# Dao-AILab/flash-attention

Measured on AMD Instinct MI355X. Metric: attention_fwd_tflops, higher is better.
Workload: dtype bf16; 1 GPU; BASELINE config 3: B=4 H=32 S=4096 D=128 bf16 causal, forward (flash_attn_func path, fa_fwd via C ABI); batch=4, heads=32, seqlen=4096, head_dim=128, causal=True, parallelism=replicas x1

## Files before the change

### flash-attention_amd/csrc/fa_api.cpp

```cpp
#include <hip/hip_runtime.h>
#include <dlfcn.h>

#include <algorithm>
#include <atomic>
#include <cmath>
#include <cstdarg>
#include <cstdio>
#include <cstdlib>
#include <cstring>
#include <initializer_list>

#include "../../include/fa_gfx950.h"
#include "fa_device.h"
#include "fa_kernel_params.h"
#include "fa_launch.h"

namespace {

thread_local char g_err[512] = {0};

int fail(int code, const char* fmt, ...) {
  va_list ap;
  va_start(ap, fmt);
  vsnprintf(g_err, sizeof(g_err), fmt, ap);
  va_end(ap);
  return code;
}

int env_int(const char* name, int dflt) {
  const char* s = getenv(name);
  return (s && *s) ? atoi(s) : dflt;
}

std::atomic<const fa::Knobs*> g_knobs{nullptr};
const fa::Knobs* read_knobs() {
  fa::Knobs* k = new fa::Knobs();
  k->fwd_nw = env_int("FA_FWD_NW", 0);
  const char* t = getenv("FA_RESCALE_THR");
  k->rescale_thr = (t && *t) ? (float)atof(t) : 8.f;
  if (!(k->rescale_thr >= 0.f) || k->rescale_thr > 16.f) k->rescale_thr = 0.f;
  k->varlen_list = env_int("FA_VARLEN_LIST", 1);
  k->il_sched = env_int("FA_IL_SCHED", 3);
  k->bwd_dq_nw = env_int("FA_BWD_DQ_NW", 0);
  k->bwd_mode = env_int("FA_BWD_MODE", 0);
  k->bwd_dkdv = env_int("FA_BWD_DKDV", 0);
  k->bwd_ds_cap_mb = env_int("FA_BWD_DS_CAP_MB", 8192);
  k->bwd_fused_check = env_int("FA_BWD_FUSED_CHECK", 0);
  k->bwd_c5_cap_mb = std::max(16, std::min(65536, env_int("FA_BWD_C5_CAP_MB", 1024)));
  k->fz_line = std::max(1, std::min(64, env_int("FA_FZ_LINE", 32)));
  k->bwd_gsplit = env_int("FA_BWD_GSPLIT", 1);
  k->w64_persist = env_int("FA_W64_PERSIST", 1);
  k->strict = env_int("FA_STRICT", 0);
  k->dkdv_prescale = env_int("FA_DKDV_PRESCALE", 0);
  k->bwd_fuse_delta = env_int("FA_BWD_FUSE_DELTA", 1);
  k->pack_gqa = env_int("FA_PACK_GQA", 1);
  k->fp8_kv_ring = env_int("FA_FP8_KV_RING", 4);
  if (k->fp8_kv_ring < 2 || k->fp8_kv_ring > 4) k->fp8_kv_ring = 4;
  k->launch_log = env_int("FA_DEBUG_LAUNCH_LOG", 0);
  if (k->strict) k->rescale_thr = 0.f;
  return k;
}

}
namespace fa {
const Knobs& knobs() {
  const Knobs* k = g_knobs.load(std::memory_order_acquire);
  if (!k) {
    const Knobs* fresh = read_knobs();
    if (g_knobs.compare_exchange_strong(k, fresh, std::memory_order_acq_rel)) k = fresh;
    else delete fresh;
  }
  return *k;
}
LastSchedule& last_schedule() {
  thread_local LastSchedule ls{};
  return ls;
}
namespace {
constexpr int kLaunchLogCap = 256;
struct LaunchLog { int n; const void* kern[kLaunchLogCap]; };
LaunchLog& launch_log() {
  thread_local LaunchLog l{};
  return l;
}
}
void launch_log_push(const void* kern) {
  LaunchLog& l = launch_log();
  if (l.n < kLaunchLogCap) l.kern[l.n] = kern;
  ++l.n;
}
void launch_log_clear() { launch_log().n = 0; }
int launch_log_count() { return launch_log().n; }
const void* launch_log_at(int i) { return (i >= 0 && i < launch_log().n && i < kLaunchLogCap) ? launch_log().kern[i] : nullptr; }
}
namespace {

bool head_dim_trimmed(int d) { return d == 32 || d == 96 || d == 192; }
bool head_dim_native(int d) { return d == 64 || d == 128 || d == 256 || head_dim_trimmed(d); }
int head_dim_kernel(int d) { for (int n : {32, 64, 96, 128, 192}) if (d <= n) return n; return 256; }
int head_dim_pitch(int d) { return d <= 64 ? 64 : d <= 128 ? 128 : 256; }

void normalize_window(int seqlen_q, int seqlen_k, bool has_alibi, int& is_causal, int& wl, int& wr) {
  if (wl >= seqlen_k) wl = -1;
  if (wr >= seqlen_k) wr = -1;
  if (seqlen_q == 1 && !has_alibi) is_causal = 0;
  if (is_causal) wr = 0;
  if (wl < 0) wl = -1;
  if (wr < 0) wr = -1;
}

int check_dropout(float p_dropout, const void* rng_state) {
  if (!(p_dropout >= 0.f) || p_dropout >= 1.f) return fail(FA_ERR_INVALID_ARGUMENT, "p_dropout must be in [0, 1)");
  if (p_dropout > 0.f && !rng_state) return fail(FA_ERR_INVALID_ARGUMENT, "p_dropout > 0 needs a device rng_state {seed, offset}");
  return FA_OK;
}
template <typename K> void fill_dropout(K& k, float p_dropout, const uint64_t* rng_state, int seqlen_k) {
  if (p_dropout > 0.f) {
    k.rng = rng_state;
    const float p_keep = 1.0f - p_dropout;
    k.drop_thr8 = (uint32_t)std::floor(p_keep * 255.0f);
    k.rp_keep = 1.f / (1.f - p_dropout);
  }
}

inline bool mla_pair(int d, int d_v) { return d == 576 && d_v == 512; }
constexpr int kMlaBlockRows = 64;
int pack_group(const FaFwdParams* a) {
  const int g = a->h_k > 0 ? a->h / a->h_k : 1;
  if (mla_pair(a->d, a->d_v)) return g > 1 ? g : 1;
  if (g <= 1 || !fa::knobs().pack_gqa || (a->d_v > 0 && a->d_v != a->d) || a->cu_seqlens_q || a->seqused_q || a->p_dropout > 0.f || a->seqlen_q < 1 || (long)a->seqlen_q * g > 128) return 1;
  return g;
}
int choose_splits(const FaFwdParams* a, int& split_tiles) {
  const int tiles = (a->seqlen_k + 63) / 64;
// ... 1076 lines not shown
```

### flash-attention_amd/csrc/fa_fwd_w64.hip

```cpp
#include <cstddef>
#include <cstdio>
#include <cstdlib>
#include <type_traits>

#include "fa_device.h"
#include "fa_kernel_params.h"
#include "fa_launch.h"
#include "fa_fwd_w64_regs.h"
#define FA_W64_CLOB FA_W64_ACC_CLOBBERS
#include "fa_w64_asm.h"


#define FA_W64_AH 3
#define FA_W64_KDMA_G0 0
#define FA_W64_KDMA_GS 2
#define FA_W64_VDMA_G0 1
#define FA_W64_VDMA_GS 2

namespace fa {

template <int D> FA_DEVINL constexpr int k_swz_w(int row) { return D == 128 ? (row & 15) : ((row >> 1) & 7); }
template <int D> FA_DEVINL constexpr int v_swz_w(int row) { return D == 128 ? (row & 3) : ((row >> 1) & 1); }

#define FA_W64_MFMA(E_) (std::is_same<E_, __bf16>::value ? "v_mfma_f32_32x32x16_bf16" : "v_mfma_f32_32x32x16_f16")
constexpr int W64_Q_BASE = 128;
template <typename E, int F> FA_DEVINL void mfma_s_first(f32x16& d, u32x4 a, const f32x16& c) {
  if constexpr (std::is_same<E, __bf16>::value)
    asm volatile("v_mfma_f32_32x32x16_bf16 %0, %1, a[%c3:%c4], %2" : "=&v"(d) : "v"(a), "v"(c), "i"(W64_Q_BASE + 4 * F), "i"(W64_Q_BASE + 4 * F + 3) : FA_W64_ACC_CLOBBERS);
  else
    asm volatile("v_mfma_f32_32x32x16_f16 %0, %1, a[%c3:%c4], %2" : "=&v"(d) : "v"(a), "v"(c), "i"(W64_Q_BASE + 4 * F), "i"(W64_Q_BASE + 4 * F + 3) : FA_W64_ACC_CLOBBERS);
}
template <typename E, int F> FA_DEVINL void mfma_s_acc(f32x16& d, u32x4 a) {
  if constexpr (std::is_same<E, __bf16>::value)
    asm volatile("v_mfma_f32_32x32x16_bf16 %0, %1, a[%c2:%c3], %0" : "+v"(d) : "v"(a), "i"(W64_Q_BASE + 4 * F), "i"(W64_Q_BASE + 4 * F + 3) : FA_W64_ACC_CLOBBERS);
  else
    asm volatile("v_mfma_f32_32x32x16_f16 %0, %1, a[%c2:%c3], %0" : "+v"(d) : "v"(a), "i"(W64_Q_BASE + 4 * F), "i"(W64_Q_BASE + 4 * F + 3) : FA_W64_ACC_CLOBBERS);
}
template <typename E, int T> FA_DEVINL void mfma_o_acc(u32x4 a, u32x4 b) {
  if constexpr (std::is_same<E, __bf16>::value)
    asm volatile("v_mfma_f32_32x32x16_bf16 a[%c2:%c3], %0, %1, a[%c2:%c3]" : : "v"(a), "v"(b), "i"(16 * T), "i"(16 * T + 15) : FA_W64_ACC_CLOBBERS);
  else
    asm volatile("v_mfma_f32_32x32x16_f16 a[%c2:%c3], %0, %1, a[%c2:%c3]" : : "v"(a), "v"(b), "i"(16 * T), "i"(16 * T + 15) : FA_W64_ACC_CLOBBERS);
}
template <typename E, int D, int FEAT = 0, bool PAGED = false, bool DENSE = false>
__global__ void __launch_bounds__(256, 1) fa_fwd_w64_kernel(const FwdK p) {
  constexpr bool ALIBI = FEAT == FEAT_ALIBI;
  static_assert(!PAGED || FEAT == 0, "the paged variant serves plain attention");
  static_assert(!DENSE || (FEAT == 0 && !PAGED), "the dense variant serves plain attention on contiguous keys / values");
  constexpr bool SOFTCAP = FEAT == FEAT_CAP;
  constexpr bool DROP = FEAT == FEAT_DROP;
  constexpr bool DESC = ALIBI;
  static_assert(FEAT == 0 || FEAT == FEAT_ALIBI || FEAT == FEAT_CAP || FEAT == FEAT_DROP, "feature variants of this schedule: none, causal ALiBi, softcap, dropout");
  using T = ElemTraits<E>;
  using V8 = typename T::v8;
  constexpr int NW = 4, QB = 2, BM = NW * 64, BN = 64, CPR = D / 8;
  constexpr int ROW_BYTES = D * 2;
  constexpr int TILE_BYTES = BN * ROW_BYTES;
  constexpr int KS = D / 16;
  constexpr int DB = D / 32;
  static_assert(D == 64 || D == 128, "head dims built natively: 64, 128");
  constexpr float kLn2 = 0.6931471805599453f;

  extern __shared__ __attribute__((aligned(16))) char smem[];
  char FA_LDS* lds = (char FA_LDS*)smem;
  constexpr int STAGE_BYTES = BM * (ROW_BYTES + 16);
  constexpr int Q_OFF = (4 * TILE_BYTES > STAGE_BYTES ? 4 * TILE_BYTES : STAGE_BYTES + 1023) / 1024 * 1024;

  const int tid = threadIdx.x;
  const int lane = tid & 63;
  const int wave = __builtin_amdgcn_readfirstlane(tid >> 6);
  const int hi = lane >> 5, qi = lane & 31;

  const int d_row = lane / CPR, d_pc = lane % CPR;
  constexpr int RPD = 1024 / ROW_BYTES;

  struct Blk { int b, h, m_block, sq, sk; int64_t q_row0, k_row0, q_boff, k_boff, v_boff, o_boff; };
  const int n_virtual = p.persist_total > 0 ? p.persist_total : (int)gridDim.x;
  auto load_rc = [&]() __attribute__((always_inline)) {
#if defined(__HIP_DEVICE_COMPILE__)
    const char __attribute__((address_space(4)))* ka = (const char __attribute__((address_space(4)))*)__builtin_amdgcn_kernarg_segment_ptr();
    asm volatile("" : "+s"(ka));
    const uint32_t __attribute__((address_space(4)))* w = (const uint32_t __attribute__((address_space(4)))*)(ka + offsetof(FwdK, rc));
    W64Rc r;
    r.mul[0] = w[0]; r.mul[1] = w[1]; r.mul[2] = w[2]; r.mul[3] = w[3]; r.mul[4] = w[4]; r.shifts = w[5];
    return r;
#else
    return p.rc;
#endif
  };
  const W64Rc rc0 = load_rc();
  const int g8 = (int)(gridDim.x >> 3);
  const bool snake = p.persist_total > 0 && p.wr >= 0 && p.unit_size > 1 && g8 - fastdiv(g8, rc_get(rc0, RC_UNIT)) * p.unit_size == 0;
  auto decode_id = [&](const W64Rc& rc, int vb, int round, Blk& k) __attribute__((always_inline)) -> bool {
    if (vb >= n_virtual) return false;
    if (!DENSE && p.work_list) {
      if (!work_list_item(p.work_list, vb, p.h, p.h_k, k.b, k.h, k.m_block)) return false;
    } else {
      if (!fwd_w64_decode(p, rc, vb, snake && (round & 1), k.b, k.h, k.m_block)) return false;
    }
    return true;
  };
  auto fill_blk = [&](Blk& k) __attribute__((always_inline)) -> bool {
    k.sq = p.sq; k.sk = p.sk; k.q_row0 = 0; k.k_row0 = 0;
    if constexpr (DENSE) {
      k.q_boff = (int64_t)k.b * p.q_bs; k.k_boff = (int64_t)k.b * p.k_bs; k.v_boff = (int64_t)k.b * p.v_bs; k.o_boff = (int64_t)k.b * p.o_bs;
      return k.m_block * BM < k.sq;
    }
    const int bkv = p.kv_batch_idx ? p.kv_batch_idx[k.b] : k.b;
    k.q_boff = (int64_t)k.b * p.q_bs; k.k_boff = (int64_t)bkv * p.k_bs; k.v_boff = (int64_t)bkv * p.v_bs; k.o_boff = (int64_t)k.b * p.o_bs;
    if (p.cu_q) { const int c0 = p.cu_q[k.b]; k.sq = p.cu_q[k.b + 1] - c0; k.q_row0 = c0; k.q_boff = 0; k.o_boff = 0; }
    if (p.seqused_q) k.sq = min(k.sq, p.seqused_q[k.b]);
    if (p.cu_k) { const int c0 = p.cu_k[k.b]; k.sk = p.cu_k[k.b + 1] - c0; k.k_row0 = c0; k.k_boff = 0; k.v_boff = 0; }
    if (p.seqused_k) k.sk = min(p.seqused_k[k.b] + p.seqused_add, (p.cu_k && !PAGED) ? k.sk : p.sk);
    if (p.leftpad_k) {
      const int lp = p.leftpad_k[k.b];
      k.sk = max(0, k.sk - lp);
      k.k_row0 += lp;
    }
    if constexpr (PAGED) { k.k_boff = 0; k.v_boff = 0; k.k_row0 = 0; }
    return k.m_block * BM < k.sq;
  };
  constexpr int QDMA = (BM * ROW_BYTES) / 1024 / NW;
  auto q_srd_of = [&](const Blk& k) __attribute__((always_inline)) {
    const E* base = (const E*)p.q + k.q_boff + (k.q_row0 + (int64_t)k.m_block * BM) * p.q_rs + (int64_t)k.h * p.q_hs;
    const int rows = min(BM, k.sq - k.m_block * BM);
    const unsigned long long a = (unsigned long long)base;
    const unsigned nrec = rows > 0 ? (unsigned)(((unsigned long long)(rows - 1) * (unsigned long long)p.q_rs + D) * 2ull) : 0u;
    const unsigned lo = __builtin_amdgcn_readfirstlane((unsigned)a);
    const unsigned hi16 = __builtin_amdgcn_readfirstlane((unsigned)(a >> 32)) & 0xffffu;
    const unsigned nr = __builtin_amdgcn_readfirstlane(nrec);
    u32x4 srd = {lo, hi16, nr, 0x00020000u};
    return srd;
  };
  auto dma_q_piece = [&](const u32x4& srd, int i) __attribute__((always_inline)) {
    const int pc = wave * QDMA + i;
    const int row = pc * RPD + d_row;
    const unsigned vo = (unsigned)(row * (int)p.q_rs + ((d_pc ^ k_swz_w<D>(row)) << 3)) * 2u;
    const unsigned dst = __builtin_amdgcn_readfirstlane((unsigned)(Q_OFF + pc * 1024));
    unsigned keep;
    asm volatile("s_mov_b32 %0, m0\n\ts_mov_b32 m0, %2\n\ts_nop 0\n\tbuffer_load_dwordx4 %1, %3, 0 offen lds\n\ts_mov_b32 m0, %0"
                 : "=&s"(keep) : "v"(vo), "s"(dst), "s"(srd) : "memory");
  };
  auto dma_q = [&](const u32x4& srd) __attribute__((always_inline)) {
#pragma unroll 1
    for (int i = 0; i < QDMA; ++i) dma_q_piece(srd, i);
  };
  int q_in_lds = -1;

  constexpr int NDMA = TILE_BYTES / 1024;
  constexpr int DPW = NDMA / NW;
  unsigned koff_l[DPW], voff_l[DPW];
#pragma unroll
  for (int i = 0; i < DPW; ++i) {
    const int row = (wave * DPW + i) * RPD + d_row;
    const int kc = d_pc ^ k_swz_w<D>(row);
    const int vc = ((((d_pc >> 2) ^ v_swz_w<D>(row)) << 2) | (d_pc & 3));
    koff_l[i] = (unsigned)(row * (int)p.k_rs + kc * 8) * 2u - (unsigned)(i * 1024);
    voff_l[i] = (unsigned)(row * (int)p.v_rs + vc * 8) * 2u - (unsigned)(i * 1024);
  }
  const float thr = p.rescale_thr;
  const bool has_wl = !DENSE && p.wl >= 0;

  Blk cur_id;
  cur_id.b = 0; cur_id.h = 0; cur_id.m_block = 0;
  bool cur_ok = decode_id(rc0, (int)blockIdx.x, 0, cur_id);
  for (int vb = blockIdx.x, round = 0; vb < n_virtual; vb += gridDim.x, ++round) {
  Blk blk = cur_id, nxt;
  const bool blk_ok = cur_ok && fill_blk(blk);
  nxt.b = 0; nxt.h = 0; nxt.m_block = 0;
  const W64Rc rc = load_rc();
  const bool nxt_id_ok = p.persist_total > 0 && decode_id(rc, vb + (int)gridDim.x, round + 1, nxt);
  cur_id.b = __builtin_amdgcn_readfirstlane(nxt.b); cur_id.h = __builtin_amdgcn_readfirstlane(nxt.h); cur_id.m_block = __builtin_amdgcn_readfirstlane(nxt.m_block);
  cur_ok = nxt_id_ok;
  if (!blk_ok) continue;
  const int b = blk.b, h = blk.h, m_block = blk.m_block, sq = blk.sq, sk = blk.sk;
  const int hk = fastdiv(h, rc_get(rc, RC_HKR));
  const int64_t q_row0 = blk.q_row0, k_row0 = blk.k_row0, q_boff = blk.q_boff, k_boff = blk.k_boff, v_boff = blk.v_boff, o_boff = blk.o_boff;
  const int m0 = m_block * BM;

  const E* __restrict__ kp = (const E*)p.k + k_boff + k_row0 * p.k_rs + (int64_t)hk * p.k_hs;
  const E* __restrict__ vp = (const E*)p.v + v_boff + k_row0 * p.v_rs + (int64_t)hk * p.v_hs;
  E* __restrict__ op = (E*)p.o + o_boff + q_row0 * p.o_rs + (int64_t)h * p.o_hs;
  float* __restrict__ lsep = (!DENSE && p.cu_q) ? (p.lse + (int64_t)h * p.total_q + q_row0) : (p.lse + ((int64_t)b * p.h + h) * p.sq);

  const int shift = sk - sq;
  const int blk_last = min(m0 + BM, sq) - 1;
  int kmax = sk - 1, kmin = 0;
  if (p.wr >= 0) kmax = min(kmax, blk_last + shift + p.wr);
  if (has_wl) kmin = max(0, m0 + shift - p.wl);
  const int n_min = kmin / BN;
  const int n_max = (kmax >= kmin) ? (kmax / BN + 1) : n_min;
  const int n_tiles = n_max - n_min;
  const int n_steps = 2 * n_tiles;
  const int key_base = n_min * BN;
  auto tile_of = [&](int u) __attribute__((always_inline)) { return DESC ? n_tiles - 1 - u : u; };
  auto step_key = [&](int i) __attribute__((always_inline)) { return key_base + BN * tile_of(i >> 1) + 32 * (i & 1); };
  float slope2 = 0.f;
  if constexpr (ALIBI) slope2 = p.alibi[(int64_t)b * p.alibi_bs + h] * 1.4426950408889634f;

  const int w_row0 = m0 + wave * 64;
  const int w_row1 = min(w_row0 + 63, sq - 1);
  const bool wave_valid = w_row0 < sq;
  const int w_kmax = (p.wr >= 0) ? min(sk - 1, w_row1 + shift + p.wr) : sk - 1;
  const int w_kmin = has_wl ? max(0, w_row0 + shift - p.wl) : 0;
  const int w_full_hi = (p.wr >= 0) ? min(sk - 1, w_row0 + shift + p.wr) : sk - 1;
  const int w_full_lo = has_wl ? (w_row1 + shift - p.wl) : 0;
  int lim_hi[QB], lim_lo[QB];
#pragma unroll
  for (int qb = 0; qb < QB; ++qb) {
    const int my_row = w_row0 + 32 * qb + qi;
    lim_hi[qb] = (p.wr >= 0) ? min(sk - 1, my_row + shift + p.wr) : sk - 1;
    lim_lo[qb] = has_wl ? max(0, my_row + shift - p.wl) : 0;
  }
  auto make_srd = [&](const void* base, int64_t row_stride) __attribute__((always_inline)) {
    const unsigned long long a = (unsigned long long)base;
    const unsigned lo = __builtin_amdgcn_readfirstlane((unsigned)a);
    const unsigned hi16 = __builtin_amdgcn_readfirstlane((unsigned)(a >> 32)) & 0xffffu;
    const unsigned long long bytes = sk > 0 ? ((unsigned long long)(sk - 1) * (unsigned long long)row_stride + D) * 2ull : 0ull;
    const unsigned nrec = __builtin_amdgcn_readfirstlane((unsigned)(bytes > 0xffffffffull ? 0xffffffffull : bytes));
    u32x4 s = {lo, hi16, nrec, 0x00020000u};
    return s;
  };
  const u32x4 k_srd = make_srd(kp, p.k_rs), v_srd = make_srd(vp, p.v_rs);
  const u32x4 null_srd = {k_srd[0], k_srd[1], 0u, k_srd[3]};
  const int pg_tpp = __builtin_amdgcn_readfirstlane(PAGED ? p.page_size / BN : 1);
  const int pg_last = __builtin_amdgcn_readfirstlane(sk > 0 ? (sk - 1) / max(p.page_size, 1) : 0);
  const int* __restrict__ pg_table = p.block_table + (PAGED ? (int64_t)__builtin_amdgcn_readfirstlane(b) * p.block_table_bs : 0);
  auto page_entry = [&](int page) __attribute__((always_inline)) {
    const int pc = min(max(page, 0), pg_last);
    return __builtin_amdgcn_readfirstlane(pg_table[pc]);
  };
  const unsigned pg_bytes_k = (unsigned)__builtin_amdgcn_readfirstlane((int)(unsigned)(p.k_bs * 2)), pg_bytes_v = (unsigned)__builtin_amdgcn_readfirstlane((int)(unsigned)(p.v_bs * 2));
  const unsigned tl_bytes_k = (unsigned)__builtin_amdgcn_readfirstlane((int)(unsigned)(BN * p.k_rs * 2)), tl_bytes_v = (unsigned)__builtin_amdgcn_readfirstlane((int)(unsigned)(BN * p.v_rs * 2));
  auto uniform64 = [](const void* ptr) __attribute__((always_inline)) {
    const unsigned long long a = (unsigned long long)ptr;
    const unsigned lo = (unsigned)__builtin_amdgcn_readfirstlane((int)(unsigned)a), hi = (unsigned)__builtin_amdgcn_readfirstlane((int)(unsigned)(a >> 32));
    return ((unsigned long long)hi << 32) | (unsigned long long)lo;
  };
  const unsigned long long pg_base_k = uniform64(kp), pg_base_v = uniform64(vp);
  auto tile_srd = [&](auto isvc, int blk, int tin, int n) __attribute__((always_inline)) {
    constexpr bool ISV = decltype(isvc)::value != 0;
    const unsigned rs = (unsigned)(ISV ? p.v_rs : p.k_rs);
    const int rows = (n >= 0) ? min(BN, sk - n * BN) : 0;
    const unsigned long long a = (ISV ? pg_base_v : pg_base_k) + (unsigned long long)(unsigned)blk * (unsigned long long)(ISV ? pg_bytes_v : pg_bytes_k) + (unsigned long long)((unsigned)tin * (ISV ? tl_bytes_v : tl_bytes_k));
    const unsigned nrec = rows > 0 ? ((unsigned)(rows - 1) * rs + (unsigned)D) * 2u : 0u;
    u32x4 sd = {(unsigned)a, (unsigned)(a >> 32) & 0xffffu, nrec, 0x00020000u};
    return sd;
  };
  auto dma_pieces = [&](const u32x4& srd, const unsigned (&vo)[DPW], unsigned lds_dst) __attribute__((always_inline)) {
    unsigned keep;
    const unsigned dst = __builtin_amdgcn_readfirstlane(lds_dst);
    if constexpr (DPW == 4) {
      asm volatile("s_mov_b32 %0, m0\n\ts_mov_b32 m0, %5\n\ts_nop 0\n\t"
                   "buffer_load_dwordx4 %1, %6, 0 offen lds\n\t"
                   "buffer_load_dwordx4 %2, %6, 0 offen offset:1024 lds\n\t"
                   "buffer_load_dwordx4 %3, %6, 0 offen offset:2048 lds\n\t"
                   "buffer_load_dwordx4 %4, %6, 0 offen offset:3072 lds\n\t"
                   "s_mov_b32 m0, %0"
                   : "=&s"(keep) : "v"(vo[0]), "v"(vo[1]), "v"(vo[2]), "v"(vo[3]), "s"(dst), "s"(srd) : "memory");
    } else {
      asm volatile("s_mov_b32 %0, m0\n\ts_mov_b32 m0, %3\n\ts_nop 0\n\t"
                   "buffer_load_dwordx4 %1, %4, 0 offen lds\n\t"
                   "buffer_load_dwordx4 %2, %4, 0 offen offset:1024 lds\n\t"
                   "s_mov_b32 m0, %0"
                   : "=&s"(keep) : "v"(vo[0]), "v"(vo[DPW - 1]), "s"(dst), "s"(srd) : "memory");
    }
  };
  auto dma_tile = [&](auto isvc, int buf, int t) __attribute__((always_inline)) {
    constexpr bool ISV = decltype(isvc)::value != 0;
    const bool real = t >= 0 && t < n_tiles;
    const int64_t rs = ISV ? p.v_rs : p.k_rs;
    const unsigned lds_dst = (unsigned)((ISV ? 2 + buf : buf) * TILE_BYTES + wave * DPW * 1024);
    if constexpr (PAGED) {
      const int n = n_min + t, page = max(n, 0) / pg_tpp;
      const u32x4 sd = real ? tile_srd(isvc, page_entry(page), max(n, 0) - page * pg_tpp, n) : null_srd;
      dma_pieces(sd, ISV ? voff_l : koff_l, lds_dst);
      return;
    }
// ... 318 lines not shown
          cap_a1[e] = __builtin_fmaf(yv, kCapTiny, capoff[e >> 4]);
          cap_d[e] = fast_exp2(yv) + 1.f;
        }
      }
#pragma unroll
      for (int e = (DO_P ? el_end(x) : 32); e < (DO_P ? el_end(x + 1) : 32); ++e) {
        const int eq = e >> 4, r = e & 15;
        pe[eq][r] = fast_exp2(s_cur[eq][r]);
        l_run[eq][r & 1] += pe[eq][r];
      }
      if constexpr (x >= QKG) {
        constexpr int y = x - QKG;
        constexpr int CPG = 16 / PVG > 0 ? 16 / PVG : 1;
#pragma unroll
        for (int c = (DO_P ? y * CPG : 16); c < (y + 1) * CPG && c < 16; ++c) {
          const int j = c >> 2, m = c & 3, cq = j >> 1, t = j & 1;
          using V2 = __attribute__((ext_vector_type(2))) E;
          V2 pr;
          float pv0 = pe[cq][8 * t + 2 * m], pv1 = pe[cq][8 * t + 2 * m + 1];
          if constexpr (DROP) {
            const int r0 = 8 * t + 2 * m;
            const unsigned w = ph_c0[4 * cq + (r0 >> 2)];
            pv0 = (((w >> (8 * (r0 & 3))) & 0xffu) > drop_thr) ? 0.f : pv0;
            pv1 = (((w >> (8 * ((r0 + 1) & 3))) & 0xffu) > drop_thr) ? 0.f : pv1;
          }
          pr[0] = (E)pv0;
          pr[1] = (E)pv1;
          unsigned pw = __builtin_bit_cast(unsigned, pr);
          asm volatile("" : "+v"(pw));
          pf_cur[cq][t][m] = pw;
        }
#pragma unroll
        for (int mq = (DO_QK ? 0 : QB); mq < QB; ++mq) {
          const int g0 = tree_g0(mq);
          if (y >= g0 && y < g0 + 8 / UPG) {
#pragma unroll
            for (int u = (y - g0) * UPG; u < (y - g0 + 1) * UPG; ++u)
              if (u == 7 && UPG == 1) {
                float t_in = tmax[mq], t_out, t_cp;
                asm volatile("v_max_f32 %0, %2, %3\n\tv_mov_b32 %1, %0" : "=&v"(t_out), "=v"(t_cp) : "v"(t_in), "v"(s_nxt[mq][15]));
                tmax[mq] = t_out; tcopy[mq] = t_cp;
              } else
              tmax[mq] = u == 0 ? vmax3(s_nxt[mq][0], s_nxt[mq][1], s_nxt[mq][2])
                                : u < 7 ? vmax3(tmax[mq], s_nxt[mq][2 * u + 1], s_nxt[mq][2 * u + 2]) : vmax2(tmax[mq], s_nxt[mq][15]);
          }
          if (y == hm_gap(mq) - 1 && UPG != 1) asm volatile("v_mov_b32 %0, %1" : "=v"(tcopy[mq]) : "v"(tmax[mq]));
          if (y == hm_gap(mq)) {
            if constexpr (!DO_PV) asm volatile("s_nop 1\n\tv_permlane32_swap_b32 %0, %1\n\tv_max_f32 %0, %0, %1" : "+v"(tmax[mq]), "+v"(tcopy[mq]));
            else asm volatile("v_permlane32_swap_b32 %0, %1\n\tv_max_f32 %0, %0, %1" : "+v"(tmax[mq]), "+v"(tcopy[mq]));
          }
          if constexpr (SOFTCAP) {
            constexpr int last = PVG - 1;
            const int g1 = hm_gap(mq) + 1 < last ? hm_gap(mq) + 1 : last, g2 = hm_gap(mq) + 2 < last ? hm_gap(mq) + 2 : last, g3 = hm_gap(mq) + 3 < last ? hm_gap(mq) + 3 : last;
            if (y == g1) cap_g[mq] = fast_exp2(tmax[mq]) + 1.f;
            if (y == g2) cap_g[mq] = __builtin_fmaf(__builtin_amdgcn_rcpf(cap_g[mq]), cap_m2c, capoff[mq]);
            if (y == g3) cap_gt[mq] = __builtin_fmaf(tmax[mq], kCapTiny, cap_g[mq]);
          }
        }
      }
      if constexpr (half == 0 && x >= NG - AH && DO_QK) {
        constexpr int fn = x - (NG - AH);
        kfr[fn % RING] = *(const u32x4 FA_LDS*)(unsigned long)(unsigned)(ka[fn] + par * TILE_BYTES + 32 * ROW_BYTES);
      }
      __builtin_amdgcn_sched_barrier(0);
    });
#pragma unroll
    for (int mq = 0; mq < QB; ++mq)
      if (hm_gap(mq) >= PVG && DO_QK) tmax[mq] = vhalf_max(tmax[mq]);
    static_assert(!SOFTCAP || QB + 8 / UPG < PVG - 1, "softcap: the capped maximum is made inside the gaps");
    if constexpr (SOFTCAP) { tmax[0] = cap_gt[0]; tmax[1] = cap_gt[1]; }
    if constexpr (MODE != 4) decide_and_rescale(tmax, s_nxt);
  };

  int u_first = n_tiles + 1, u_last = n_tiles, p_lo = n_tiles + 1, p_hi = n_tiles;
  if (wave_valid && n_tiles > 0) {
    const int a_lo = max(0, (w_kmin - key_base) >> 5);
    const int a_hi = min(n_steps - 1, (w_kmax - key_base) >> 5);
    if (a_hi >= a_lo) {
      u_first = a_lo >> 1; u_last = min(n_tiles, (a_hi + 2) >> 1);
      const int f_lo = max(0, (w_full_lo - key_base + 31) >> 5);
      const int f_hi = (w_full_hi - 31 - key_base) >> 5;
      p_lo = max(u_first, (f_lo + 1) >> 1);
      p_hi = min(u_last, (f_hi - 1) >> 1);
      if constexpr (DESC) {
        const int t_lo = a_lo >> 1, t_hi = a_hi >> 1, pl_t = (f_lo + 1) >> 1, ph_t = (f_hi - 1) >> 1;
        u_first = n_tiles - 1 - t_hi; u_last = n_tiles - t_lo;
        p_lo = max(u_first, n_tiles - 1 - ph_t);
        p_hi = min(u_last, n_tiles - 1 - pl_t);
      }
      if (p_hi < p_lo) { p_lo = u_last + 1; p_hi = u_last; }
    }
  }
  u_first = __builtin_amdgcn_readfirstlane(u_first); u_last = __builtin_amdgcn_readfirstlane(u_last);
  const unsigned wave_dst = (unsigned)(wave * DPW * 1024);
  auto iter_end = [&]() __attribute__((always_inline)) {
    lds_dma_wait_all();
    __syncthreads();
  };
  const int m_lo = __builtin_amdgcn_readfirstlane(p_lo), m_hi = __builtin_amdgcn_readfirstlane(p_hi);
  const unsigned step_k = (unsigned)(BN * 2) * (unsigned)p.k_rs, step_v = (unsigned)(BN * 2) * (unsigned)p.v_rs;
  const int nmin_s = __builtin_amdgcn_readfirstlane(n_min), nts_s = __builtin_amdgcn_readfirstlane(n_tiles);
  int pg_blk_k = 0, pg_tin_k = 0, pg_blk_v = 0, pg_tin_v = 0, pg_page_n = 0, pg_tin_n = 0;
  auto pg_enter = [&](int u) __attribute__((always_inline)) {
    if constexpr (PAGED) {
      const int nv = n_min + u, nk = nv + 1, nn = nv + 2;
      pg_tin_v = nv % pg_tpp; pg_blk_v = page_entry(nv / pg_tpp);
      pg_tin_k = nk % pg_tpp; pg_blk_k = page_entry(nk / pg_tpp);
      pg_page_n = nn / pg_tpp; pg_tin_n = nn - pg_page_n * pg_tpp;
    }
  };
  auto step_pair = [&](auto parc, int u, auto pmc) __attribute__((always_inline)) {
    constexpr int par = decltype(parc)::value, PM = decltype(pmc)::value;
    using M0 = ICw<(PM == 1 ? 1 : PM == 2 ? 3 : 0)>; using M1 = ICw<(PM == 1 ? 2 : PM == 2 ? 4 : 0)>;
    q_trickle();
    u32x4 kring[FA_W64_AH + 1];
    const int us = __builtin_amdgcn_readfirstlane(u);
    unsigned dst_k = (unsigned)((par ^ 1) * TILE_BYTES) + wave_dst, dst_v = (unsigned)((2 + par) * TILE_BYTES) + wave_dst;
    unsigned tk_ = (unsigned)(nmin_s + (DESC ? nts_s - 2 - us : us + 1)) * step_k, tv_ = (unsigned)(nmin_s + (DESC ? nts_s - 1 - us : us)) * step_v;
    int im32 = ((us - m_lo) | (m_hi - us)) >> 31;
    dst_k = __builtin_amdgcn_readfirstlane(dst_k); dst_v = __builtin_amdgcn_readfirstlane(dst_v);
    im32 = __builtin_amdgcn_readfirstlane(im32);
    u32x4 srd_k = k_srd, srd_v = v_srd;
    if constexpr (PAGED) {
      const int bk = __builtin_amdgcn_readfirstlane(pg_blk_k), tk = __builtin_amdgcn_readfirstlane(pg_tin_k);
      const int bv = __builtin_amdgcn_readfirstlane(pg_blk_v), tv = __builtin_amdgcn_readfirstlane(pg_tin_v);
      const int pn = __builtin_amdgcn_readfirstlane(pg_page_n), tn = __builtin_amdgcn_readfirstlane(pg_tin_n);
      srd_k = tile_srd(ICw<0>{}, bk, tk, nmin_s + us + 1);
      srd_v = tile_srd(ICw<1>{}, bv, tv, nmin_s + us);
      tk_ = 0u; tv_ = 0u;
      pg_blk_v = bk; pg_tin_v = tk;
      pg_blk_k = page_entry(pn); pg_tin_k = tn;
      const bool wrap = tn + 1 == pg_tpp;
      pg_tin_n = wrap ? 0 : tn + 1;
      pg_page_n = wrap ? pn + 1 : pn;
    }
    asm volatile("" : "+s"(tk_), "+s"(tv_), "+s"(dst_k), "+s"(dst_v), "+s"(im32));
    auto masked = [&]() __attribute__((always_inline)) { int c = im32; asm volatile("" : "+s"(c)); return c != 0; };
    if constexpr (PM != 2) { if (__builtin_expect(masked(), 0)) set_mask(2 * u); }
    fast_step(ICw<0>{}, parc, sA, sB, pfA, pfB, srd_k, koff_l, tk_, dst_k, kring, DROP ? step_key(2 * us - 1) >> 2 : 0, M0{});
    if constexpr (PM != 2) { if (__builtin_expect(masked(), 0)) set_mask(2 * u + 1); }
    fast_step(ICw<1>{}, parc, sB, sA, pfB, pfA, srd_v, voff_l, tv_, dst_v, kring, DROP ? step_key(2 * us) >> 2 : 0, M1{});
    if constexpr (PM != 2) {
      if (__builtin_expect(masked(), 0)) {
        int to_last = FEAT == 0 ? u_last - 1 - us : 1;
        asm volatile("" : "+s"(to_last));
        if (to_last != 0) clear_mask(2 * u + 2);
      }
    }
    iter_end();
  };
  auto idle_iter = [&](int u) __attribute__((always_inline)) {
    q_trickle();
    dma_tile(ICw<0>{}, (u & 1) ^ 1, tile_of(u + 1)); dma_tile(ICw<1>{}, u & 1, tile_of(u));
    iter_end();
  };
  if (n_tiles > 0) {
    const bool active = u_first <= u_last;
    const int ua = active ? (u_first & ~1) : n_tiles + 1;
    int u = 0;
#pragma unroll 1
    for (; u < ua; ++u) idle_iter(u);
    if (active) {
      pg_enter(u);
      if constexpr (ALIBI) { if (u > 0) clear_mask(2 * u); }
      if constexpr (FEAT == 0) {
        step_pair(ICw<0>{}, u, ICw<1>{}); ++u;
#pragma unroll 1
        for (;;) {
          if (u >= u_last) break;
          step_pair(ICw<1>{}, u, ICw<0>{}); ++u;
          if (u >= u_last) break;
          step_pair(ICw<0>{}, u, ICw<0>{}); ++u;
        }
        if (u & 1) step_pair(ICw<1>{}, u, ICw<2>{}); else step_pair(ICw<0>{}, u, ICw<2>{});
        ++u;
      } else {
#pragma unroll 1
        for (;;) {
          step_pair(ICw<0>{}, u, ICw<0>{}); ++u;
          if (u > u_last) break;
          step_pair(ICw<1>{}, u, ICw<0>{}); ++u;
          if (u > u_last) break;
        }
      }
    }
#pragma unroll 1
    for (; u <= n_tiles; ++u) idle_iter(u);
  }

  if (wave_valid) {
  mfma_drain_acc();
  u32x4 o_srd;
  {
    const int rows = min(BM, sq - m0);
    const unsigned long long a = (unsigned long long)(op + (int64_t)m0 * p.o_rs);
    const unsigned lo = __builtin_amdgcn_readfirstlane((unsigned)a);
    const unsigned hi16 = __builtin_amdgcn_readfirstlane((unsigned)(a >> 32)) & 0xffffu;
    const unsigned nr = __builtin_amdgcn_readfirstlane((unsigned)(((unsigned long long)(rows - 1) * (unsigned long long)p.o_rs + D) * 2ull));
    o_srd = u32x4{lo, hi16, nr, 0x00020000u};
  }
  static_for<QB>([&](auto qbc) __attribute__((always_inline)) {
    constexpr int qb = decltype(qbc)::value;
    f32x16 o_v[DB];
    static_for<DB>([&](auto dbc) __attribute__((always_inline)) {
      constexpr int db = decltype(dbc)::value;
      acc_read_tuple<16 * (qb * DB + db)>(o_v[db]);
    });
    const float l_tot = half_sum(l_run[qb][0] + l_run[qb][1]);
    const bool dead = (l_tot == 0.f) || (l_tot != l_tot);
    const float inv = (dead ? 1.f : 1.f / l_tot) * o_lag[qb] * (DROP ? p.rp_keep : 1.f);
    const int row0 = w_row0 + 32 * qb;
    if (row0 < sq) {
      {
        using V4 = typename T::v4;
        constexpr int RS = ROW_BYTES + 16, RPI = 64 / CPR;
        char FA_LDS* stage = lds + (wave * 64 + qb * 32) * RS;
#pragma unroll
        for (int db = 0; db < DB; ++db)
#pragma unroll
          for (int g = 0; g < 4; ++g) {
            V4 ov;
#pragma unroll
            for (int jj = 0; jj < 4; ++jj) ov[jj] = (E)(o_v[db][4 * g + jj] * inv);
            *reinterpret_cast<V4 FA_LDS*>(stage + qi * RS + (32 * db + 8 * g + 4 * hi) * 2) = ov;
          }
        unsigned lane_off = (unsigned)(((wave * 64 + lane / CPR) * (int)p.o_rs + (lane % CPR) * 8) * 2);
        asm volatile("" : "+v"(lane_off));
#pragma unroll
        for (int i = 0; i < 32 / RPI; ++i) {
          const u32x4 x = *reinterpret_cast<const u32x4 FA_LDS*>(stage + (i * RPI + lane / CPR) * RS + (lane % CPR) * 16);
          const unsigned soff = __builtin_amdgcn_readfirstlane((unsigned)((qb * 32 + i * RPI) * (int)p.o_rs * 2));
          asm volatile("buffer_store_dwordx4 %0, %1, %2, %3 offen" : : "v"(x), "v"(lane_off), "s"(o_srd), "s"(soff) : "memory");
        }
        asm volatile("s_waitcnt lgkmcnt(0)" ::: "memory");
      }
      const int my_row = row0 + qi;
      if (my_row < sq && hi == 0) lsep[my_row] = dead ? INFINITY : (m_run[qb] * kLn2 + __logf(l_tot));
    }
  });
  }
  }
}

template <typename E, int D, int FEAT = 0, bool PAGED = false, bool DENSE = false>
static int launch_fwd_w64_t(const FwdK& p, hipStream_t stream) {
  if constexpr (FEAT == 0 && !PAGED && !DENSE) {
    if (!p.cu_q && !p.cu_k && !p.seqused_q && !p.seqused_k && !p.leftpad_k && !p.kv_batch_idx && !p.work_list && p.wl < 0)
      return launch_fwd_w64_t<E, D, 0, false, true>(p, stream);
  }
  constexpr int STAGE = 256 * (D * 2 + 16);
  constexpr int smem = ((4 * 64 * D * 2 > STAGE ? 4 * 64 * D * 2 : STAGE + 1023) / 1024 * 1024) + 256 * D * 2;
  auto kern = fa_fwd_w64_kernel<E, D, FEAT, PAGED, DENSE>;
  static std::atomic<unsigned long long> attr_mask{0};
  if (ensure_dyn_lds(attr_mask, (const void*)kern, smem, true) != 0) return -1;
  const long long total = p.work_list ? (long long)p.work_bound * p.h : units_grid(p.n_units, p.unit_size);
  if (total <= 0) return 0;
  FwdK pp = p;
  fwd_w64_reciprocals(pp);
  long long grid = total;
  const int cus = device_cu_count();
  const bool balanced = p.wr < 0 || (p.unit_size > 1 && (cus / 8) % p.unit_size == 0);
  if (!p.work_list && cus >= 8 && total > cus && balanced && knobs().w64_persist != 0) {
    grid = cus / 8 * 8;
    pp.persist_total = (int)total;
  }
  FA_LAUNCH(kern, dim3((unsigned)grid), dim3(256), smem, stream, pp);
  if (hipGetLastError() != hipSuccess) return -1;
  LastSchedule& ls = last_schedule();
  ls.fwd_kernel = 3; ls.fwd_nw = 4; ls.fwd_feat = FEAT; ls.fwd_splits = 1; ls.fwd_list = p.work_list != nullptr; ls.d = D;
  ls.bf16 = std::is_same<E, __bf16>::value;
  if (FEAT) snprintf(ls.name, sizeof(ls.name), "fa::fa_fwd_w64_kernel<%s,%d,%s>", ls.bf16 ? "bf16" : "f16", D, FEAT == FEAT_CAP ? "softcap" : FEAT == FEAT_DROP ? "dropout" : "alibi");
  else if (PAGED) snprintf(ls.name, sizeof(ls.name), "fa::fa_fwd_w64_kernel<%s,%d,paged>", ls.bf16 ? "bf16" : "f16", D);
  else if (DENSE) snprintf(ls.name, sizeof(ls.name), "fa::fa_fwd_w64_kernel<%s,%d,dense>", ls.bf16 ? "bf16" : "f16", D);
  else snprintf(ls.name, sizeof(ls.name), "fa::fa_fwd_w64_kernel<%s,%d>", ls.bf16 ? "bf16" : "f16", D);
  return 0;
}

#ifndef FA_W64_PART
#define FA_W64_PART 0
#endif
int launch_fwd_w64_bf16(const FwdK& p, int d, hipStream_t stream);
int launch_fwd_w64_f16(const FwdK& p, int d, hipStream_t stream);
#if FA_W64_PART != 1
int launch_fwd_w64_f16(const FwdK& p, int d, hipStream_t stream) {
  if (p.rng) {
    if (d == 128) return launch_fwd_w64_t<_Float16, 128, FEAT_DROP>(p, stream);
    if (d == 64) return launch_fwd_w64_t<_Float16, 64, FEAT_DROP>(p, stream);
    return -2;
  }
  if (p.softcap > 0.f) {
    if (d == 128) return launch_fwd_w64_t<_Float16, 128, FEAT_CAP>(p, stream);
    if (d == 64) return launch_fwd_w64_t<_Float16, 64, FEAT_CAP>(p, stream);
    return -2;
  }
  if (p.alibi) {
    if (d == 128) return launch_fwd_w64_t<_Float16, 128, FEAT_ALIBI>(p, stream);
    if (d == 64) return launch_fwd_w64_t<_Float16, 64, FEAT_ALIBI>(p, stream);
    return -2;
  }
  if (p.block_table) {
    if (d == 128) return launch_fwd_w64_t<_Float16, 128, 0, true>(p, stream);
    if (d == 64) return launch_fwd_w64_t<_Float16, 64, 0, true>(p, stream);
    return -2;
  }
  if (d == 128) return launch_fwd_w64_t<_Float16, 128>(p, stream);
  if (d == 64) return launch_fwd_w64_t<_Float16, 64>(p, stream);
  return -2;
}
#endif
#if FA_W64_PART != 2
int launch_fwd_w64_bf16(const FwdK& p, int d, hipStream_t stream) {
  if (p.rng) {
    if (d == 128) return launch_fwd_w64_t<__bf16, 128, FEAT_DROP>(p, stream);
    if (d == 64) return launch_fwd_w64_t<__bf16, 64, FEAT_DROP>(p, stream);
    return -2;
  }
  if (p.softcap > 0.f) {
    if (d == 128) return launch_fwd_w64_t<__bf16, 128, FEAT_CAP>(p, stream);
    if (d == 64) return launch_fwd_w64_t<__bf16, 64, FEAT_CAP>(p, stream);
    return -2;
  }
  if (p.alibi) {
    if (d == 128) return launch_fwd_w64_t<__bf16, 128, FEAT_ALIBI>(p, stream);
    if (d == 64) return launch_fwd_w64_t<__bf16, 64, FEAT_ALIBI>(p, stream);
    return -2;
  }
  if (p.block_table) {
    if (d == 128) return launch_fwd_w64_t<__bf16, 128, 0, true>(p, stream);
    if (d == 64) return launch_fwd_w64_t<__bf16, 64, 0, true>(p, stream);
    return -2;
  }
  if (d == 128) return launch_fwd_w64_t<__bf16, 128>(p, stream);
  if (d == 64) return launch_fwd_w64_t<__bf16, 64>(p, stream);
  return -2;
}
int launch_fwd_w64(const FwdK& p, int dtype_bf16, int d, hipStream_t stream) {
  if (p.n_splits > 1) return -2;
  if (p.rng != nullptr && (p.randval != nullptr || p.softcap > 0.f || p.alibi != nullptr || p.block_table != nullptr)) return -2;
  if (p.softcap > 0.f && p.alibi != nullptr) return -2;
  if (p.block_table != nullptr && (p.softcap > 0.f || p.alibi != nullptr || p.leftpad_k != nullptr || p.kv_batch_idx != nullptr || p.page_size % 64 != 0)) return -2;
  if (p.block_table != nullptr && ((uint64_t)(p.k_bs > p.v_bs ? p.k_bs : p.v_bs) * 2u >= (1ull << 32) || (uint64_t)p.page_size * (uint64_t)(p.k_rs > p.v_rs ? p.k_rs : p.v_rs) * 2u >= (1ull << 32))) return -2;
// ... 10 lines not shown
```

### flash-attention_amd/csrc/fa_kernel_params.h

```cpp
#pragma once
#include <stdint.h>
#include <hip/hip_runtime.h>

namespace fa {

struct FastDiv { uint32_t mul, shift; };
inline FastDiv fastdiv_make(int32_t d) {
  FastDiv f = {0x80000000u, 0u};
  if (d <= 1) return f;
  while ((1ull << f.shift) < (uint64_t)d) ++f.shift;
  f.mul = (uint32_t)(((1ull << (31 + f.shift)) + (uint64_t)d - 1) / (uint64_t)d);
  return f;
}
#if defined(__HIPCC__)
__host__ __device__
#endif
inline int32_t fastdiv(int32_t n, FastDiv f) { return (int32_t)((uint32_t)(((uint64_t)((uint32_t)n << 1) * (uint64_t)f.mul) >> 32) >> f.shift); }
enum { RC_UNIT = 0, RC_HPX = 1, RC_NMB = 2, RC_H = 3, RC_HKR = 4 };
struct alignas(8) W64Rc { uint32_t mul[5]; uint32_t shifts; };
#if defined(__HIPCC__)
__host__ __device__
#endif
inline FastDiv rc_get(const W64Rc& r, int i) { FastDiv f = {r.mul[i], (r.shifts >> (6 * i)) & 63u}; return f; }

struct FwdK {
  const void* q;
  const void* k;
  const void* v;
  void* o;
  float* lse;
  int64_t q_bs, q_rs, q_hs;
  int64_t k_bs, k_rs, k_hs;
  int64_t v_bs, v_rs, v_hs;
  int64_t o_bs, o_rs, o_hs;
  const int32_t* cu_q;
  const int32_t* cu_k;
  const int32_t* seqused_k;
  const int32_t* seqused_q;
  const int32_t* kv_batch_idx;
  const int32_t* block_table;
  int64_t block_table_bs;
  int32_t page_size;
  int32_t seqused_add;
  const int32_t* leftpad_k;
  const float* alibi;
  int64_t alibi_bs;
  int32_t b, h, h_k, hk_ratio;
  int32_t sq, sk;
  int32_t total_q;
  int32_t nmb;
  int32_t n_units, unit_size, unit_hpx;
  int32_t wl, wr;
  float scale;
  float scale_log2;
  float softcap;
  float rescale_thr;
  int32_t pack_g;
  int32_t d_chunks;
  int32_t persist_total;
  int32_t work_bound;
  const int2* work_list;
  int32_t n_splits, split_tiles;
  float* o_accum;
  float* lse_accum;
  const uint64_t* rng;
  uint8_t* randval;
  int64_t rv_bs, rv_hs, rv_rs;
  uint32_t drop_thr8;
  float rp_keep;
  W64Rc rc;
};
#if defined(__HIPCC__)
__host__ __device__
#endif
inline bool fwd_w64_decode(const FwdK& p, const W64Rc& rc, int32_t vb, bool mirror, int32_t& b, int32_t& h, int32_t& m_block) {
  const int32_t xcd = vb & 7, slot = vb >> 3;
  const int32_t j = fastdiv(slot, rc_get(rc, RC_UNIT));
  int32_t item = slot - j * p.unit_size;
  if (mirror) item = p.unit_size - 1 - item;
  int32_t unit = xcd + 8 * j;
  if (p.unit_hpx > 0) {
    const int32_t bb = fastdiv(j, rc_get(rc, RC_HPX));
    unit = bb * (8 * p.unit_hpx) + xcd * p.unit_hpx + (j - bb * p.unit_hpx);
  }
  if (unit >= p.n_units) return false;
  const int32_t w = unit * p.unit_size + item;
  const int32_t bh = fastdiv(w, rc_get(rc, RC_NMB));
  const int32_t mbr = w - bh * p.nmb;
  m_block = (p.wr >= 0) ? (p.nmb - 1 - mbr) : mbr;
  b = fastdiv(bh, rc_get(rc, RC_H));
  h = bh - b * p.h;
  return true;
}
inline void fwd_w64_reciprocals(FwdK& k) {
  const int32_t d[5] = {k.unit_size, k.unit_hpx, k.nmb, k.h, k.hk_ratio};
  k.rc.shifts = 0u;
  for (int i = 0; i < 5; ++i) { const FastDiv f = fastdiv_make(d[i]); k.rc.mul[i] = f.mul; k.rc.shifts |= f.shift << (6 * i); }
}

struct Fp8K {
  const float* q_descale;
  const float* k_descale;
  const float* v_descale;
  int64_t q_bs, q_hs, k_bs, k_hs, v_bs, v_hs;
};

enum { FZ_ERR = 0, FZ_STATS = 32, FZ_CTRL = 64, FZ_CTRL_STRIDE = 160, FZ_TAIL = 0, FZ_HEAD = 32, FZ_AVAIL = 64, FZ_DONE = 96, FZ_NEXT = 128, FZ_COUNTERS = FZ_CTRL + 8 * FZ_CTRL_STRIDE };
inline constexpr long long fz_sync_words(long long items, int line) { return FZ_COUNTERS + items * line + 8 * items; }

struct BwdK {
  const void* dout;
  const void* q;
  const void* k;
  const void* v;
  const void* o;
  const float* lse;
  void* dq;
  void* dk;
  void* dv;
  float* delta;
  int64_t do_bs, do_rs, do_hs;
  int64_t q_bs, q_rs, q_hs;
  int64_t k_bs, k_rs, k_hs;
  int64_t v_bs, v_rs, v_hs;
  int64_t o_bs, o_rs, o_hs;
  int64_t dq_bs, dq_rs, dq_hs;
  int64_t dk_bs, dk_rs, dk_hs;
  int64_t dv_bs, dv_rs, dv_hs;
  const int32_t* cu_q;
  const int32_t* cu_k;
  const int32_t* seqused_q;
  const int32_t* seqused_k;
  const float* alibi;
  int64_t alibi_bs;
  int32_t b, h, h_k, hk_ratio;
  int32_t sq, sk;
  int32_t total_q, total_k;
  int32_t nmb, nnb;
  int32_t q_units, q_unit_size, q_unit_hpx;
  int32_t k_units, k_unit_size, k_unit_hpx;
  int32_t wl, wr;
  float scale;
  float scale_log2;
  float softcap;
  int32_t q_bound, k_bound;
  const int2* q_list;
  const int2* k_list;
  const uint64_t* rng;
  uint32_t drop_thr8;
  float rp_keep;
  void* ds_ws;
  int32_t ds_nq32, ds_nk32;
// ... 20 lines not shown
```

### flash-attention_amd/csrc/fa_launch.h

```cpp
#pragma once
#include <hip/hip_runtime.h>
#include <atomic>
#include "fa_kernel_params.h"

namespace fa {

struct Knobs {
  int fwd_nw;
  float rescale_thr;
  int varlen_list;
  int il_sched;
  int bwd_dq_nw;
  int bwd_dkdv;
  int bwd_mode;
  int bwd_c5_cap_mb;
  int bwd_gsplit;
  int fz_line;
  int bwd_ds_cap_mb;
  int bwd_fused_check;
  int w64_persist;
  int pack_gqa;
  int dkdv_prescale;
  int bwd_fuse_delta;
  int fp8_kv_ring;
  int launch_log;
  int strict;
};
const Knobs& knobs();

struct LastSchedule {
  int fwd_kernel;
  int fwd_nw;
  int fwd_feat;
  int fwd_splits;
  int fwd_list;
  int d, bf16;
  int bwd_dq_nw, bwd_list, bwd_spill;
  int fwd_pack;
  int bwd_dkdv_nw;
  int dv;
  char name[96];
};
LastSchedule& last_schedule();

void launch_log_push(const void* kern);
void launch_log_clear();
int launch_log_count();
const void* launch_log_at(int i);
template <typename K> inline void launch_log_note(K kern) {
  if (__builtin_expect(knobs().launch_log != 0, 0)) launch_log_push(reinterpret_cast<const void*>(kern));
}
#define FA_LAUNCH(kern, grid, block, smem, stream, ...) \
  do {                                                  \
    ::fa::launch_log_note(kern);                        \
    hipLaunchKernelGGL(kern, grid, block, smem, stream, __VA_ARGS__); \
  } while (0)

inline int device_cu_count() {
  static std::atomic<int> cache[64];
  int dev = 0;
  if (hipGetDevice(&dev) != hipSuccess) return 0;
  int v = dev < 64 ? cache[dev].load(std::memory_order_relaxed) : 0;
  if (v == 0) {
    if (hipDeviceGetAttribute(&v, hipDeviceAttributeMultiprocessorCount, dev) != hipSuccess) return 0;
    if (dev < 64) cache[dev].store(v, std::memory_order_relaxed);
  }
  return v;
}

inline int ensure_dyn_lds(std::atomic<unsigned long long>& mask, const void* kern, int smem, bool need_base0 = false) {
  int dev = 0;
  if (hipGetDevice(&dev) != hipSuccess) return -1;
  const unsigned long long bit = 1ull << (dev & 63);
  if (dev < 64 && (mask.load(std::memory_order_acquire) & bit)) return 0;
  if (hipFuncSetAttribute(kern, hipFuncAttributeMaxDynamicSharedMemorySize, smem) != hipSuccess) return -1;
  if (need_base0) {
    hipFuncAttributes fattr;
    if (hipFuncGetAttributes(&fattr, kern) != hipSuccess || fattr.sharedSizeBytes != 0) return -1;
  }
  if (dev < 64) mask.fetch_or(bit, std::memory_order_release);
  return 0;
}

inline void choose_units(int batch, int kv_heads, int heads_per_group, int blocks_per_head, int& n_units, int& unit_size, int& hpx) {
  const int n_groups = batch * kv_heads;
  hpx = 0;
  if (kv_heads % 8 == 0) { n_units = n_groups; unit_size = heads_per_group * blocks_per_head; hpx = kv_heads / 8; return; }
  auto ok = [](int n) { return n >= 16 && ((n + 7) / 8 * 8 - n) * 8 <= n; };
  if (ok(n_groups)) { n_units = n_groups; unit_size = heads_per_group * blocks_per_head; return; }
  const int n_heads = n_groups * heads_per_group;
  if (ok(n_heads)) { n_units = n_heads; unit_size = blocks_per_head; return; }
  n_units = n_heads * blocks_per_head; unit_size = 1;
}
inline long long units_grid(int n_units, int unit_size) { return (long long)((n_units + 7) / 8) * 8 * unit_size; }

int launch_fwd(const FwdK& p, int dtype_bf16, int d, int nw, hipStream_t stream);
int fwd_block_m(int nw);

struct KvAppendK {
  const void* knew; const void* vnew; void* kcache; void* vcache;
  int64_t kn_bs, kn_rs, kn_hs, vn_bs, vn_rs, vn_hs, kc_bs, kc_rs, kc_hs, vc_bs, vc_rs, vc_hs;
  const int32_t* seqlens_k; const int32_t* kv_batch_idx; const int32_t* block_table; int64_t block_table_bs;
  int32_t page_size, b, s_new, h_k, d;
// ... 42 lines not shown
```

Before: 1113 TFLOP/s.

## Add optional descending key-tile walk for causal w64 forward kernel

Adds a runtime knob (FA_W64_WALK, off by default) that lets the plain causal w64 forward kernel walk key tiles in descending order, with the diagonal masked tile processed first. To support this, tile offsets become a base plus a signed stride, and the masking-branch hints change for that path. The main loop is also restructured so it can start at an odd tile (no longer rounding u_first down to even), using a lim_a bound to realign the parity. That part runs by default and may trim one idle iteration per block, at the cost of an extra branch in the hot loop.

```diff
diff --git a/flash-attention_amd/csrc/fa_api.cpp b/flash-attention_amd/csrc/fa_api.cpp
--- a/flash-attention_amd/csrc/fa_api.cpp
+++ b/flash-attention_amd/csrc/fa_api.cpp
@@ -50,6 +50,7 @@
   k->fz_line = std::max(1, std::min(64, env_int("FA_FZ_LINE", 32)));
   k->bwd_gsplit = env_int("FA_BWD_GSPLIT", 1);
   k->w64_persist = env_int("FA_W64_PERSIST", 1);
+  k->w64_walk = env_int("FA_W64_WALK", 0);
   k->strict = env_int("FA_STRICT", 0);
   k->dkdv_prescale = env_int("FA_DKDV_PRESCALE", 0);
   k->bwd_fuse_delta = env_int("FA_BWD_FUSE_DELTA", 1);
diff --git a/flash-attention_amd/csrc/fa_fwd_w64.hip b/flash-attention_amd/csrc/fa_fwd_w64.hip
--- a/flash-attention_amd/csrc/fa_fwd_w64.hip
+++ b/flash-attention_amd/csrc/fa_fwd_w64.hip
@@ -50,6 +50,7 @@
   constexpr bool SOFTCAP = FEAT == FEAT_CAP;
   constexpr bool DROP = FEAT == FEAT_DROP;
   constexpr bool DESC = ALIBI;
+  constexpr bool WALK_RT = FEAT == 0 && !PAGED;
   static_assert(FEAT == 0 || FEAT == FEAT_ALIBI || FEAT == FEAT_CAP || FEAT == FEAT_DROP, "feature variants of this schedule: none, causal ALiBi, softcap, dropout");
   using T = ElemTraits<E>;
   using V8 = typename T::v8;
@@ -159,6 +160,7 @@
     voff_l[i] = (unsigned)(row * (int)p.v_rs + vc * 8) * 2u - (unsigned)(i * 1024);
   }
   const float thr = p.rescale_thr;
+  const bool desc = DESC || (WALK_RT && __builtin_amdgcn_readfirstlane(p.w64_walk_down) != 0);
   const bool has_wl = !DENSE && p.wl >= 0;
 
   Blk cur_id;
@@ -193,7 +195,7 @@
   const int n_tiles = n_max - n_min;
   const int n_steps = 2 * n_tiles;
   const int key_base = n_min * BN;
-  auto tile_of = [&](int u) __attribute__((always_inline)) { return DESC ? n_tiles - 1 - u : u; };
+  auto tile_of = [&](int u) __attribute__((always_inline)) { return desc ? n_tiles - 1 - u : u; };
   auto step_key = [&](int i) __attribute__((always_inline)) { return key_base + BN * tile_of(i >> 1) + 32 * (i & 1); };
   float slope2 = 0.f;
   if constexpr (ALIBI) slope2 = p.alibi[(int64_t)b * p.alibi_bs + h] * 1.4426950408889634f;
@@ -678,7 +680,7 @@
       const int f_hi = (w_full_hi - 31 - key_base) >> 5;
       p_lo = max(u_first, (f_lo + 1) >> 1);
       p_hi = min(u_last, (f_hi - 1) >> 1);
-      if constexpr (DESC) {
+      if (desc) {
         const int t_lo = a_lo >> 1, t_hi = a_hi >> 1, pl_t = (f_lo + 1) >> 1, ph_t = (f_hi - 1) >> 1;
         u_first = n_tiles - 1 - t_hi; u_last = n_tiles - t_lo;
         p_lo = max(u_first, n_tiles - 1 - ph_t);
@@ -696,6 +698,9 @@
   const int m_lo = __builtin_amdgcn_readfirstlane(p_lo), m_hi = __builtin_amdgcn_readfirstlane(p_hi);
   const unsigned step_k = (unsigned)(BN * 2) * (unsigned)p.k_rs, step_v = (unsigned)(BN * 2) * (unsigned)p.v_rs;
   const int nmin_s = __builtin_amdgcn_readfirstlane(n_min), nts_s = __builtin_amdgcn_readfirstlane(n_tiles);
+  const int desc_m = desc ? -1 : 0;
+  const unsigned tk0_s = (unsigned)(nmin_s + (desc ? nts_s - 2 : 1)) * step_k, tv0_s = (unsigned)(nmin_s + (desc ? nts_s - 1 : 0)) * step_v;
+  const unsigned dstep_k = desc ? 0u - step_k : step_k, dstep_v = desc ? 0u - step_v : step_v;
   int pg_blk_k = 0, pg_tin_k = 0, pg_blk_v = 0, pg_tin_v = 0, pg_page_n = 0, pg_tin_n = 0;
   auto pg_enter = [&](int u) __attribute__((always_inline)) {
     if constexpr (PAGED) {
@@ -712,8 +717,11 @@
     u32x4 kring[FA_W64_AH + 1];
     const int us = __builtin_amdgcn_readfirstlane(u);
     unsigned dst_k = (unsigned)((par ^ 1) * TILE_BYTES) + wave_dst, dst_v = (unsigned)((2 + par) * TILE_BYTES) + wave_dst;
-    unsigned tk_ = (unsigned)(nmin_s + (DESC ? nts_s - 2 - us : us + 1)) * step_k, tv_ = (unsigned)(nmin_s + (DESC ? nts_s - 1 - us : us)) * step_v;
+    unsigned tk_ = WALK_RT ? tk0_s + (unsigned)us * dstep_k : (unsigned)(nmin_s + (DESC ? nts_s - 2 - us : us + 1)) * step_k;
+    unsigned tv_ = WALK_RT ? tv0_s + (unsigned)us * dstep_v : (unsigned)(nmin_s + (DESC ? nts_s - 1 - us : us)) * step_v;
     int im32 = ((us - m_lo) | (m_hi - us)) >> 31;
+    constexpr bool FIRST_RT = WALK_RT && PM == 1;
+    if constexpr (FIRST_RT) im32 |= desc_m;
     dst_k = __builtin_amdgcn_readfirstlane(dst_k); dst_v = __builtin_amdgcn_readfirstlane(dst_v);
     im32 = __builtin_amdgcn_readfirstlane(im32);
     u32x4 srd_k = k_srd, srd_v = v_srd;
@@ -732,12 +740,12 @@
     }
     asm volatile("" : "+s"(tk_), "+s"(tv_), "+s"(dst_k), "+s"(dst_v), "+s"(im32));
     auto masked = [&]() __attribute__((always_inline)) { int c = im32; asm volatile("" : "+s"(c)); return c != 0; };
-    if constexpr (PM != 2) { if (__builtin_expect(masked(), 0)) set_mask(2 * u); }
+    if constexpr (PM != 2) { if (__builtin_expect(masked(), FIRST_RT ? 1 : 0)) set_mask(2 * u); }
     fast_step(ICw<0>{}, parc, sA, sB, pfA, pfB, srd_k, koff_l, tk_, dst_k, kring, DROP ? step_key(2 * us - 1) >> 2 : 0, M0{});
-    if constexpr (PM != 2) { if (__builtin_expect(masked(), 0)) set_mask(2 * u + 1); }
+    if constexpr (PM != 2) { if (__builtin_expect(masked(), FIRST_RT ? 1 : 0)) set_mask(2 * u + 1); }
     fast_step(ICw<1>{}, parc, sB, sA, pfB, pfA, srd_v, voff_l, tv_, dst_v, kring, DROP ? step_key(2 * us) >> 2 : 0, M1{});
     if constexpr (PM != 2) {
-      if (__builtin_expect(masked(), 0)) {
+      if (__builtin_expect(masked(), FIRST_RT ? 1 : 0)) {
         int to_last = FEAT == 0 ? u_last - 1 - us : 1;
         asm volatile("" : "+s"(to_last));
         if (to_last != 0) clear_mask(2 * u + 2);
@@ -752,7 +760,7 @@
   };
   if (n_tiles > 0) {
     const bool active = u_first <= u_last;
-    const int ua = active ? (u_first & ~1) : n_tiles + 1;
+    const int ua = active ? (FEAT == 0 ? u_first : (u_first & ~1)) : n_tiles + 1;
     int u = 0;
 #pragma unroll 1
     for (; u < ua; ++u) idle_iter(u);
@@ -760,12 +768,17 @@
       pg_enter(u);
       if constexpr (ALIBI) { if (u > 0) clear_mask(2 * u); }
       if constexpr (FEAT == 0) {
-        step_pair(ICw<0>{}, u, ICw<1>{}); ++u;
+        int lim_a = u_last;
+        if (u & 1) { step_pair(ICw<1>{}, u, ICw<1>{}); ++u; lim_a = u; } else { step_pair(ICw<0>{}, u, ICw<1>{}); ++u; }
 #pragma unroll 1
         for (;;) {
-          if (u >= u_last) break;
-          step_pair(ICw<1>{}, u, ICw<0>{}); ++u;
-          if (u >= u_last) break;
+          if (__builtin_expect(u >= lim_a, 0)) {
+            if (u >= u_last) break;
+            lim_a = u_last;
+          } else {
+            step_pair(ICw<1>{}, u, ICw<0>{}); ++u;
+            if (u >= u_last) break;
+          }
           step_pair(ICw<0>{}, u, ICw<0>{}); ++u;
         }
         if (u & 1) step_pair(ICw<1>{}, u, ICw<2>{}); else step_pair(ICw<0>{}, u, ICw<2>{});
@@ -853,6 +866,7 @@
   if (total <= 0) return 0;
   FwdK pp = p;
   fwd_w64_reciprocals(pp);
+  pp.w64_walk_down = (FEAT == 0 && !PAGED && p.wr >= 0 && p.wl < 0 && knobs().w64_walk != 0) ? 1 : 0;
   long long grid = total;
   const int cus = device_cu_count();
   const bool balanced = p.wr < 0 || (p.unit_size > 1 && (cus / 8) % p.unit_size == 0);
diff --git a/flash-attention_amd/csrc/fa_kernel_params.h b/flash-attention_amd/csrc/fa_kernel_params.h
--- a/flash-attention_amd/csrc/fa_kernel_params.h
+++ b/flash-attention_amd/csrc/fa_kernel_params.h
@@ -68,6 +68,7 @@
   int64_t rv_bs, rv_hs, rv_rs;
   uint32_t drop_thr8;
   float rp_keep;
+  int32_t w64_walk_down;
   W64Rc rc;
 };
 #if defined(__HIPCC__)
diff --git a/flash-attention_amd/csrc/fa_launch.h b/flash-attention_amd/csrc/fa_launch.h
--- a/flash-attention_amd/csrc/fa_launch.h
+++ b/flash-attention_amd/csrc/fa_launch.h
@@ -19,6 +19,7 @@
   int bwd_ds_cap_mb;
   int bwd_fused_check;
   int w64_persist;
+  int w64_walk;
   int pack_gqa;
   int dkdv_prescale;
   int bwd_fuse_delta;
```

New measurement: 1107 TFLOP/s. About the same (-0.6%).
